# lms-07/LGTEUN

Hardware: AMD Instinct MI355X
Metric: train image-pairs/sec, GF-2 4-band 128x128, K=4, bs=32/GPU (higher is better)
Workload: dtype f32 (GEMMs and the local mixer: split 16-bit MFMA -- f16 pairs in the forward FFN, the W2 products of its backward and P V, bf16 triples elsewhere -- fp32 accumulate; fp32-equivalent); 1 GPU; BASELINE configs[1]: C=4, MS 32x32, PAN 128x128, K=4, 32 pairs/GPU, train step = fwd + L1 + bwd + Adam + StepLR tick; mode=faithful, global_batch=32, parallelism=dp1, dropout=True

## Files before the change

### lgteun_amd/csrc/k_ffn_bwd_x.hip

```cpp
#include "kernels.h"
#include "bwd_kernels.h"
#include "split_bf16.h"
#include "hstore.h"

#ifdef LG_STAMPS
__device__ unsigned long long g_kb_stamps[4 * 16];
#define STAMP(i) do { if (blockIdx.x == 0 && lane == 0 && stamp_on) g_kb_stamps[wave * 16 + (i)] = __builtin_amdgcn_s_memtime(); } while (0)
extern "C" __attribute__((visibility("default"))) int lg_debug_kb_stamps(unsigned long long* host) {
    return (int)hipMemcpyFromSymbol(host, HIP_SYMBOL(g_kb_stamps), sizeof(g_kb_stamps));
}
#else
#define STAMP(i) do { } while (0)
#endif

namespace {

constexpr int NPX = 64;
template <int E>
struct KB {
    static constexpr int N1 = 4 * E, NW = N1 / 16, NT = 64 * NW, LPP = E / 4;
    static constexpr int LDP = N1 + 16;
    static constexpr int D2_PIECE = NPX * LDP;
    static constexpr int XN_PIECE = NPX * E;
    static constexpr int D1T_PIECE = 16 * 16;
    static constexpr size_t OFF_XN = (size_t)3 * D2_PIECE * 2;
    static constexpr size_t OFF_D1T = OFF_XN + (size_t)3 * XN_PIECE * 2;
    static constexpr size_t OFF_RED = OFF_D1T + (size_t)NW * 3 * D1T_PIECE * 2;
    static constexpr size_t LDS_BYTES = OFF_RED + (size_t)NW * NPX * E * 4;
    static constexpr int R_B2 = N1 * N1, R_W1 = R_B2 + N1, R_B1 = R_W1 + N1 * E, R_LG = R_B1 + N1, R_LB = R_LG + E, ROW = R_LB + E;
    static_assert(OFF_XN % 16 == 0 && OFF_D1T % 16 == 0 && OFF_RED % 16 == 0, "16-byte aligned LDS regions");
    static_assert(NT / (N1 / 4) == 16 && NT / LPP == NPX, "loader / LayerNorm thread maps");
};

typedef __attribute__((address_space(3))) s16x4_t lds_s16x4_t;
#ifndef LG_KB_DACHAINS
#define LG_KB_DACHAINS 0
#endif
#ifndef LG_KB_STAGGER
#define LG_KB_STAGGER 0
#endif
#ifndef LG_KB_FENCE
#define LG_KB_FENCE 1
#endif
#define KB_FENCE() do { if (LG_KB_FENCE) __builtin_amdgcn_sched_barrier(0); } while (0)

__device__ __forceinline__ float quad_sum(float v) {
    v += __builtin_bit_cast(float, __builtin_amdgcn_mov_dpp(__builtin_bit_cast(int, v), 0xB1, 0xF, 0xF, true));
    v += __builtin_bit_cast(float, __builtin_amdgcn_mov_dpp(__builtin_bit_cast(int, v), 0x4E, 0xF, 0xF, true));
    return v;
}
__device__ __forceinline__ bf16x8_t lds_x8(const uint16_t* p) { return __builtin_bit_cast(bf16x8_t, *reinterpret_cast<const u32x4_t*>(p)); }
__device__ __forceinline__ s16x4_t lds_x4(const uint16_t* p) { return __builtin_bit_cast(s16x4_t, *reinterpret_cast<const u32x2_t*>(p)); }
__device__ __forceinline__ s16x4_t lds_tr4(const uint16_t* p) {
    return __builtin_amdgcn_ds_read_tr16_b64_v4i16((lds_s16x4_t*)p);
}
__device__ __forceinline__ void mfma6_16(f32x4_t& acc, const s16x4_t (&a)[3], const s16x4_t (&b)[3]) {
    acc = __builtin_amdgcn_mfma_f32_16x16x16bf16_1k(a[0], b[2], acc, 0, 0, 0);
    acc = __builtin_amdgcn_mfma_f32_16x16x16bf16_1k(a[2], b[0], acc, 0, 0, 0);
    acc = __builtin_amdgcn_mfma_f32_16x16x16bf16_1k(a[1], b[1], acc, 0, 0, 0);
    acc = __builtin_amdgcn_mfma_f32_16x16x16bf16_1k(a[0], b[1], acc, 0, 0, 0);
    acc = __builtin_amdgcn_mfma_f32_16x16x16bf16_1k(a[1], b[0], acc, 0, 0, 0);
    acc = __builtin_amdgcn_mfma_f32_16x16x16bf16_1k(a[0], b[0], acc, 0, 0, 0);
}
__device__ __forceinline__ void mfma6_32(f32x4_t& acc, const bf16x8_t (&a)[3], const bf16x8_t (&b)[3]) {
    acc = __builtin_amdgcn_mfma_f32_16x16x32_bf16(a[0], b[2], acc, 0, 0, 0);
    acc = __builtin_amdgcn_mfma_f32_16x16x32_bf16(a[2], b[0], acc, 0, 0, 0);
    acc = __builtin_amdgcn_mfma_f32_16x16x32_bf16(a[1], b[1], acc, 0, 0, 0);
    acc = __builtin_amdgcn_mfma_f32_16x16x32_bf16(a[0], b[1], acc, 0, 0, 0);
    acc = __builtin_amdgcn_mfma_f32_16x16x32_bf16(a[1], b[0], acc, 0, 0, 0);
    acc = __builtin_amdgcn_mfma_f32_16x16x32_bf16(a[0], b[0], acc, 0, 0, 0);
}
__device__ __forceinline__ bf16x8_t cat8(s16x4_t lo, s16x4_t hi) {
    typedef short s16x8_t __attribute__((ext_vector_type(8)));
    return __builtin_bit_cast(bf16x8_t, (s16x8_t)__builtin_shufflevector(lo, hi, 0, 1, 2, 3, 4, 5, 6, 7));
}
#ifndef LG_KB_PAIR
#define LG_KB_PAIR 1
#endif
__device__ __forceinline__ void mfma3_16(f32x4_t& acc, const s16x4_t (&a)[3], const s16x4_t (&b)[3]) {
    const bf16x8_t b31 = cat8(b[2], b[0]), b21 = cat8(b[1], b[0]);
    acc = __builtin_amdgcn_mfma_f32_16x16x32_bf16(cat8(a[0], a[2]), b31, acc, 0, 0, 0);
    acc = __builtin_amdgcn_mfma_f32_16x16x32_bf16(cat8(a[1], a[1]), b21, acc, 0, 0, 0);
    acc = __builtin_amdgcn_mfma_f32_16x16x32_bf16(cat8(a[0], a[0]), b21, acc, 0, 0, 0);
}
template <int NP>
__device__ __forceinline__ void mfmaN_16(f32x4_t& acc, const s16x4_t (&a)[3], const s16x4_t (&b)[3]) {
    if (NP == 3) { if (LG_KB_PAIR) mfma3_16(acc, a, b); else mfma6_16(acc, a, b); }
    else if (NP == 2) {
        const s16x4_t z = {0, 0, 0, 0};
        acc = sb_mfma_h(cat8(a[1], a[0]), cat8(b[0], b[1]), acc);
        acc = sb_mfma_h(cat8(a[0], z), cat8(b[0], z), acc);
    } else acc = __builtin_amdgcn_mfma_f32_16x16x16bf16_1k(a[0], b[0], acc, 0, 0, 0);
}
template <int NP>
__device__ __forceinline__ void mfmaN_32(f32x4_t& acc, const bf16x8_t (&a)[3], const bf16x8_t (&b)[3]) {
    if (NP == 3) mfma6_32(acc, a, b);
    else if (NP == 2) {
        acc = sb_mfma_h(a[1], b[0], acc);
        acc = sb_mfma_h(a[0], b[1], acc);
        acc = sb_mfma_h(a[0], b[0], acc);
    } else acc = __builtin_amdgcn_mfma_f32_16x16x32_bf16(a[0], b[0], acc, 0, 0, 0);
}
template <int NP>
__device__ __forceinline__ void split4(const float (&v)[4], s16x4_t (&p)[3]) {
    u32x2_t q1, q2, q3;
    split_x4<NP>(v, q1, q2, q3);
    p[0] = __builtin_bit_cast(s16x4_t, q1); p[1] = __builtin_bit_cast(s16x4_t, q2); p[2] = __builtin_bit_cast(s16x4_t, q3);
}

template <int NP>
__device__ __forceinline__ void ld3_x4(const uint16_t* p, int piece, s16x4_t (&o)[3]) {
    o[0] = lds_x4(p);
    if (NP == 3) { o[1] = lds_x4(p + piece); o[2] = lds_x4(p + 2 * piece); } else if (NP == 2) { o[1] = lds_x4(p + piece); o[2] = o[0]; } else { o[1] = o[0]; o[2] = o[0]; }
}
template <int NP>
__device__ __forceinline__ void ld3_x8(const uint16_t* p, int piece, bf16x8_t (&o)[3]) {
    o[0] = lds_x8(p);
    if (NP == 3) { o[1] = lds_x8(p + piece); o[2] = lds_x8(p + 2 * piece); } else if (NP == 2) { o[1] = lds_x8(p + piece); o[2] = o[0]; } else { o[1] = o[0]; o[2] = o[0]; }
}
template <int NP>
__device__ __forceinline__ void ld3_tr(const uint16_t* p, int piece, s16x4_t (&o)[3]) {
    o[0] = lds_tr4(p);
    if (NP == 3) { o[1] = lds_tr4(p + piece); o[2] = lds_tr4(p + 2 * piece); } else if (NP == 2) { o[1] = lds_tr4(p + piece); o[2] = o[0]; } else { o[1] = o[0]; o[2] = o[0]; }
}
template <int NP>
__device__ __forceinline__ WFrag32 wfrag32(const float* W, int K, int kb, float ws) { return NP == 3 ? load_wfrag32(W, K, kb) : (NP == 2 ? load_wfrag32_h2(W, K, kb, ws) : load_wfrag32_rne(W, K, kb)); }
template <int NP>
__device__ __forceinline__ WFrag16 wfrag16(const float* W, int K, int k0, float ws) { return NP == 3 ? load_wfrag16(W, K, k0) : (NP == 2 ? load_wfrag16_h2(W, K, k0, ws) : load_wfrag16_rne(W, K, k0)); }
__device__ __forceinline__ float kb_pow2_below(float bound) { return __builtin_amdgcn_ldexpf(1.0f, 15 - __builtin_amdgcn_frexp_expf(bound)); }

template <int E, int NP>
__global__ __launch_bounds__(KB<E>::NT) __attribute__((amdgpu_waves_per_eu(2))) void k_ffn1_bwd_xs(Ffn1BwdXArgs a, long ntiles, int uneven) {
    using C = KB<E>;
    constexpr int N1 = C::N1, NW = C::NW, NT = C::NT, LDP = C::LDP, LPP = C::LPP, D2_PIECE = C::D2_PIECE, XN_PIECE = C::XN_PIECE, D1T_PIECE = C::D1T_PIECE;
    constexpr int KB2 = N1 / 32;
    constexpr int NE = E / 16;
    constexpr bool BF = (NP == 1);
    constexpr int NPE = NP == 2 ? 3 : NP;
    extern __shared__ __attribute__((aligned(16))) unsigned char smem_raw[];
    uint16_t* D2 = reinterpret_cast<uint16_t*>(smem_raw);
    uint16_t* XN = reinterpret_cast<uint16_t*>(smem_raw + C::OFF_XN);
    const int wave = threadIdx.x >> 6, lane = threadIdx.x & 63, r = lane & 15, g = lane >> 4;
    uint16_t* D1T = reinterpret_cast<uint16_t*>(smem_raw + C::OFF_D1T) + wave * 3 * D1T_PIECE;
    float* red = reinterpret_cast<float*>(smem_raw + C::OFF_RED);

    float S_a1 = 1.f, S_w2 = 1.f, S_d2 = 1.f;
    if constexpr (NP == 2) {
        S_a1 = a.scales[1]; S_w2 = a.scales[4];
        S_d2 = kb_pow2_below(fmaxf(a.scales[6], 8.6736174e-19f));
    }
    const float c_d1 = 1.0f / (S_d2 * S_w2);
    WFrag16 w1f16;
    WFrag32 w1f32;
    if constexpr (E == 16) w1f16 = wfrag16<NPE>(a.w1 + (size_t)(wave * 16) * E, E, 0, 1.0f);
    else w1f32 = wfrag32<NPE>(a.w1 + (size_t)(wave * 16) * E, E, 0, 1.0f);
    WFrag32 w2f[KB2];
#pragma unroll
    for (int kb = 0; kb < KB2; ++kb) w2f[kb] = wfrag32<NP>(a.w2t + (size_t)(wave * 16) * N1, N1, kb, S_w2);
    WFrag16 w1tf[NE];
#pragma unroll
    for (int rb = 0; rb < NE; ++rb) w1tf[rb] = wfrag16<NPE>(a.w1t + (size_t)(rb * 16) * N1, N1, wave * 16, 1.0f);
    const float b1s = a.b1[wave * 16 + r];
    const int lpx = threadIdx.x / LPP, lq = threadIdx.x % LPP;
    const float4 lng = *reinterpret_cast<const float4*>(a.ln2g + 4 * lq), lnb = *reinterpret_cast<const float4*>(a.ln2b + 4 * lq);
    const int dq = threadIdx.x % (N1 / 4), dpx = threadIdx.x / (N1 / 4);

    f32x4_t acc2[NW], acc1[NE];
#pragma unroll
    for (int nb = 0; nb < NW; ++nb) acc2[nb] = (f32x4_t){0.f, 0.f, 0.f, 0.f};
#pragma unroll
    for (int cb = 0; cb < NE; ++cb) acc1[cb] = (f32x4_t){0.f, 0.f, 0.f, 0.f};
    float bs1 = 0.f;
    float4 bs2 = make_float4(0.f, 0.f, 0.f, 0.f);
    float4 pg = make_float4(0.f, 0.f, 0.f, 0.f), pb = pg;

    typename HS<BF>::raw4 d2n[4];
    float4 xnx, dyn;
    auto issue = [&](long tile_) {
        const long p0 = tile_ * NPX;
#pragma unroll
        for (int it = 0; it < 4; ++it) d2n[it] = HS<BF>::ldraw(a.dh2, (p0 + dpx + 16 * it) * N1 + 4 * dq);
        xnx = *reinterpret_cast<const float4*>(a.x + (p0 + lpx) * E + 4 * lq);
        dyn = *reinterpret_cast<const float4*>(a.dy + (p0 + lpx) * E + 4 * lq);
    };
    const int half = (int)gridDim.x >> 1, first = (int)blockIdx.x < half ? 1 : 0;
    const long per = uneven ? ntiles / (8 * (long)gridDim.x) : 0;
    const long nmine = uneven ? per * (first ? uneven : 16 - uneven) : (1l << 60);
    const long t0 = uneven ? (first ? (long)blockIdx.x : (long)half * per * uneven + ((long)blockIdx.x - half)) : (long)blockIdx.x;
    const long tstep = uneven ? half : (long)gridDim.x;
    if (t0 < ntiles) issue(t0);

#pragma unroll 1
    for (long tile = t0, kt = 0; tile < ntiles && kt < nmine; tile += tstep, ++kt) {
        const long p0 = tile * NPX;
#ifdef LG_STAMPS
        const bool stamp_on = kt == 2;
#endif
        STAMP(0);
#pragma unroll
        for (int it = 0; it < 4; ++it) {
            const float4 d = HS<BF>::widen(d2n[it]);
            bs2.x += d.x; bs2.y += d.y; bs2.z += d.z; bs2.w += d.w;
            uint16_t* dst = D2 + (dpx + 16 * it) * LDP + 4 * dq;
            if constexpr (BF) {
                *reinterpret_cast<u32x2_t*>(dst) = __builtin_bit_cast(u32x2_t, d2n[it]);
            } else {
                const float v[4] = {d.x * S_d2, d.y * S_d2, d.z * S_d2, d.w * S_d2};
                u32x2_t q1, q2, q3;
                split_x4<NP>(v, q1, q2, q3);
                *reinterpret_cast<u32x2_t*>(dst) = q1;
                *reinterpret_cast<u32x2_t*>(dst + D2_PIECE) = q2;
                if (NP == 3) *reinterpret_cast<u32x2_t*>(dst + 2 * D2_PIECE) = q3;
            }
        }
        const float4 xv = xnx, dyv = dyn;
        const float mu = lane_group_sum<LPP>((xv.x + xv.y) + (xv.z + xv.w)) * (1.0f / E);
        const float c0 = xv.x - mu, c1 = xv.y - mu, c2 = xv.z - mu, c3 = xv.w - mu;
        const float rstd = __builtin_amdgcn_rsqf(lane_group_sum<LPP>((c0 * c0 + c1 * c1) + (c2 * c2 + c3 * c3)) * (1.0f / E) + LG_EPS);
        const float xh[4] = {c0 * rstd, c1 * rstd, c2 * rstd, c3 * rstd};
        {
            const float yv[4] = {xh[0] * lng.x + lnb.x, xh[1] * lng.y + lnb.y, xh[2] * lng.z + lnb.z, xh[3] * lng.w + lnb.w};
            u32x2_t q1, q2, q3;
            split_x4<NPE>(yv, q1, q2, q3);
            uint16_t* dst = XN + lpx * E + 4 * lq;
            *reinterpret_cast<u32x2_t*>(dst) = q1;
            if (NPE == 3) {
                *reinterpret_cast<u32x2_t*>(dst + XN_PIECE) = q2;
                *reinterpret_cast<u32x2_t*>(dst + 2 * XN_PIECE) = q3;
            }
        }
        if (tile + tstep < ntiles && kt + 1 < nmine) issue(tile + tstep);
        STAMP(1);
        __syncthreads();
        STAMP(2);
#if LG_KB_STAGGER
        if (NW == 8 && wave >= 4) __builtin_amdgcn_s_sleep(LG_KB_STAGGER);
#endif

#pragma unroll 1
        for (int pbk = 0; pbk < NPX / 16; ++pbk) {
            f32x4_t h1 = (f32x4_t){b1s, b1s, b1s, b1s};
            if constexpr (E == 16) {
                s16x4_t xa[3];
                ld3_x4<NPE>(XN + (pbk * 16 + r) * E + 4 * g, XN_PIECE, xa);
                KB_FENCE();
                mfmaN_16<NPE>(h1, xa, w1f16.p);
            } else {
                bf16x8_t xa[3];
                ld3_x8<NPE>(XN + (pbk * 16 + r) * E + 8 * g, XN_PIECE, xa);
                KB_FENCE();
                mfmaN_32<NPE>(h1, xa, w1f32.p);
            }
            f32x4_t da = (f32x4_t){0.f, 0.f, 0.f, 0.f};
            {
                const uint16_t* pd = D2 + (pbk * 16 + r) * LDP + 8 * g;
#if LG_KB_DACHAINS
                f32x4_t dak[KB2];
#pragma unroll
                for (int kb = 0; kb < KB2; ++kb) {
                    dak[kb] = (f32x4_t){0.f, 0.f, 0.f, 0.f};
                    bf16x8_t dk[3];
                    ld3_x8<NP>(pd + 32 * kb, D2_PIECE, dk);
                    mfmaN_32<NP>(dak[kb], dk, w2f[kb].p);
                }
#pragma unroll
                for (int kb = 0; kb < KB2; ++kb) da += dak[kb];
#else
#pragma unroll
                for (int kb = 0; kb < KB2; ++kb) {
                    bf16x8_t dk[3];
                    ld3_x8<NP>(pd + 32 * kb, D2_PIECE, dk);
                    mfmaN_32<NP>(da, dk, w2f[kb].p);
                }
#endif
            }
            KB_FENCE();
            lg_v2f a01, a23, g01, g23;
            gelu2_both_t<NP == 1>((lg_v2f){h1[0], h1[1]}, a01, g01);
            gelu2_both_t<NP == 1>((lg_v2f){h1[2], h1[3]}, a23, g23);
            if (NP == 2) { a01 *= S_a1; a23 *= S_a1; g01 *= c_d1; g23 *= c_d1; }
            const float a1v[4] = {a01.x, a01.y, a23.x, a23.y};
            const float d1v[4] = {da[0] * g01.x, da[1] * g01.y, da[2] * g23.x, da[3] * g23.y};
            bs1 += (d1v[0] + d1v[1]) + (d1v[2] + d1v[3]);
            s16x4_t a1p[3], d1p[3];
            split4<NP>(a1v, a1p);
            split4<NPE>(d1v, d1p);
            KB_FENCE();
            {
                const uint16_t* px = XN + (pbk * 16 + 4 * g + (r >> 2)) * E + 4 * (r & 3);
#pragma unroll
                for (int cb = 0; cb < NE; ++cb) {
                    s16x4_t xt[3];
                    ld3_tr<NPE>(px + 16 * cb, XN_PIECE, xt);
                    mfmaN_16<NPE>(acc1[cb], d1p, xt);
                }
                const uint16_t* pt = D2 + (pbk * 16 + 4 * g + (r >> 2)) * LDP + 4 * (r & 3);
#pragma unroll
                for (int nb = 0; nb < NW; ++nb) {
                    s16x4_t dt[3];
                    ld3_tr<NP>(pt + 16 * nb, D2_PIECE, dt);
                    mfmaN_16<NP>(acc2[nb], dt, a1p);
                }
            }
            KB_FENCE();
            {
                uint16_t* dst = D1T + r * 16 + 4 * g;
                *reinterpret_cast<u32x2_t*>(dst) = __builtin_bit_cast(u32x2_t, d1p[0]);
                if (NPE == 3) {
                    *reinterpret_cast<u32x2_t*>(dst + D1T_PIECE) = __builtin_bit_cast(u32x2_t, d1p[1]);
                    *reinterpret_cast<u32x2_t*>(dst + 2 * D1T_PIECE) = __builtin_bit_cast(u32x2_t, d1p[2]);
                }
                __builtin_amdgcn_fence(__ATOMIC_RELEASE, "wavefront");
                __builtin_amdgcn_wave_barrier();
                s16x4_t dtp[3];
                ld3_tr<NPE>(D1T + (4 * g + (r >> 2)) * 16 + 4 * (r & 3), D1T_PIECE, dtp);
#pragma unroll
                for (int rb = 0; rb < NE; ++rb) {
                    f32x4_t o = (f32x4_t){0.f, 0.f, 0.f, 0.f};
                    mfmaN_16<NPE>(o, w1tf[rb].p, dtp);
                    *reinterpret_cast<float4*>(red + ((size_t)wave * NPX + pbk * 16 + r) * E + 16 * rb + 4 * g) = make_float4(o[0], o[1], o[2], o[3]);
                }
                __builtin_amdgcn_wave_barrier();
            }
        }
        STAMP(3);
        __syncthreads();
        STAMP(4);

        {
            const float* rp = red + (size_t)lpx * E + 4 * lq;
            float dl[4] = {0.f, 0.f, 0.f, 0.f};
#pragma unroll
            for (int w2 = 0; w2 < NW; w2 += 2) {
                const float4 s0 = *reinterpret_cast<const float4*>(rp + (size_t)w2 * NPX * E), s1 = *reinterpret_cast<const float4*>(rp + (size_t)(w2 + 1) * NPX * E);
                dl[0] += s0.x + s1.x; dl[1] += s0.y + s1.y; dl[2] += s0.z + s1.z; dl[3] += s0.w + s1.w;
            }
            pg.x += dl[0] * xh[0]; pg.y += dl[1] * xh[1]; pg.z += dl[2] * xh[2]; pg.w += dl[3] * xh[3];
            pb.x += dl[0]; pb.y += dl[1]; pb.z += dl[2]; pb.w += dl[3];
            const float dxh[4] = {dl[0] * lng.x, dl[1] * lng.y, dl[2] * lng.z, dl[3] * lng.w};
            const float m1 = lane_group_sum<LPP>((dxh[0] + dxh[1]) + (dxh[2] + dxh[3])) * (1.0f / E);
            const float m2 = lane_group_sum<LPP>((dxh[0] * xh[0] + dxh[1] * xh[1]) + (dxh[2] * xh[2] + dxh[3] * xh[3])) * (1.0f / E);
            *reinterpret_cast<float4*>(a.dx + (p0 + lpx) * E + 4 * lq) =
                make_float4(dyv.x + rstd * (dxh[0] - m1 - xh[0] * m2), dyv.y + rstd * (dxh[1] - m1 - xh[1] * m2),
                            dyv.z + rstd * (dxh[2] - m1 - xh[2] * m2), dyv.w + rstd * (dxh[3] - m1 - xh[3] * m2));
        }
        STAMP(5);
    }

    float* row = a.slab + (size_t)blockIdx.x * C::ROW;
    const float inv_w2 = 1.0f / (S_d2 * S_a1);
#pragma unroll
    for (int nb = 0; nb < NW; ++nb)
#pragma unroll
        for (int v = 0; v < 4; ++v) row[(16 * nb + 4 * g + v) * N1 + 16 * wave + r] = acc2[nb][v] * inv_w2;
#pragma unroll
    for (int cb = 0; cb < NE; ++cb)
#pragma unroll
        for (int v = 0; v < 4; ++v) row[C::R_W1 + (16 * wave + 4 * g + v) * E + 16 * cb + r] = acc1[cb][v];
    {
        float s = bs1;
        s += __shfl_xor(s, 16);
        s += __shfl_xor(s, 32);
        if (g == 0) row[C::R_B1 + 16 * wave + r] = s;
    }
    __syncthreads();
    float* sc = reinterpret_cast<float*>(smem_raw);
    *reinterpret_cast<float4*>(sc + dpx * N1 + 4 * dq) = bs2;
    *reinterpret_cast<float4*>(sc + 16 * N1 + lpx * E + 4 * lq) = pg;
    *reinterpret_cast<float4*>(sc + 16 * N1 + NPX * E + lpx * E + 4 * lq) = pb;
    __syncthreads();
    if (threadIdx.x < N1) {
        float s = 0.f;
#pragma unroll
        for (int k = 0; k < 16; ++k) s += sc[k * N1 + threadIdx.x];
        row[C::R_B2 + threadIdx.x] = s;
    } else if (threadIdx.x < N1 + 2 * E) {
        const int i = threadIdx.x - N1, which = i / E, c = i % E;
        const float* src = sc + 16 * N1 + which * NPX * E + c;
        float s = 0.f;
        for (int k = 0; k < NPX; ++k) s += src[k * E];
        row[(which ? C::R_LB : C::R_LG) + c] = s;
    }
}

template <int E>
int launch_t(const Ffn1BwdXArgs& a, hipStream_t s) {
    using C = KB<E>;
    static DeviceOnce attr_once;
    if (attr_once.need()) {
        hipError_t e = hipFuncSetAttribute((const void*)k_ffn1_bwd_xs<E, 3>, hipFuncAttributeMaxDynamicSharedMemorySize, (int)C::LDS_BYTES);
        if (e == hipSuccess) e = hipFuncSetAttribute((const void*)k_ffn1_bwd_xs<E, 1>, hipFuncAttributeMaxDynamicSharedMemorySize, (int)C::LDS_BYTES);
        if (e == hipSuccess) e = hipFuncSetAttribute((const void*)k_ffn1_bwd_xs<E, 2>, hipFuncAttributeMaxDynamicSharedMemorySize, (int)C::LDS_BYTES);
        if (e != hipSuccess) { lg_set_error("ffn1_bwd_xs: hipFuncSetAttribute: %s", hipGetErrorString(e)); return (int)e; }
        attr_once.done();
    }
    const long ntiles = a.P / NPX;
    const int cap = ffn1_bwd_x_wgs(E);
    const int grid = (int)(ntiles < cap ? ntiles : cap);
#ifndef LG_FFN1B_UNEVEN
#define LG_FFN1B_UNEVEN 9
#endif
    const int uneven = (E == 16 && grid == 512 && ntiles % (8 * (long)grid) == 0 && LG_FFN1B_UNEVEN != 8) ? LG_FFN1B_UNEVEN : 0;
    if (a.hbf) k_ffn1_bwd_xs<E, 1><<<grid, C::NT, C::LDS_BYTES, s>>>(a, ntiles, uneven);
    else if (a.scales) k_ffn1_bwd_xs<E, 2><<<grid, C::NT, C::LDS_BYTES, s>>>(a, ntiles, uneven);
    else k_ffn1_bwd_xs<E, 3><<<grid, C::NT, C::LDS_BYTES, s>>>(a, ntiles, uneven);
    LG_CHECK_LAUNCH();
    ReduceJob j;
    j.dst2 = nullptr; j.nslices = grid; j.slice_stride = C::ROW;
    auto job = [&](int off, float* dst, int rows, int cols) {
        j.slab = a.slab + off; j.dst = dst; j.rows = rows; j.cols = cols; j.row_stride = cols; j.ld = cols; j.rows_valid = rows; j.cols_valid = cols;
        return launch_reduce_job(j, s);
    };
    int rc = job(0, a.d_w2, C::N1, C::N1);
    if (!rc) rc = job(C::R_B2, a.d_b2, 1, C::N1);
    if (!rc) rc = job(C::R_W1, a.d_w1, C::N1, E);
    if (!rc) rc = job(C::R_B1, a.d_b1, 1, C::N1);
    if (!rc) rc = job(C::R_LG, a.d_ln2g, 1, E);
    if (!rc) rc = job(C::R_LB, a.d_ln2b, 1, E);
    return rc;
}

}

size_t ffn1_bwd_x_slab_floats(int e) { return (size_t)ffn1_bwd_x_wgs(e) * (e == 16 ? KB<16>::ROW : KB<32>::ROW); }

int launch_ffn1_bwd_xs(int e, const Ffn1BwdXArgs& a, hipStream_t s) {
    ProfScope prof__(LG_K_FFN1_BWD, s);
    if (e != 16 && e != 32) { lg_set_error("ffn1_bwd_xs: e=%d unsupported", e); return -1; }
    if (a.P <= 0 || a.P % NPX) { lg_set_error("ffn1_bwd_xs: pixel count %ld is not a multiple of %d", a.P, NPX); return -2; }
    if (!a.dh2 || !a.x || !a.dy || !a.dx || !a.slab || !a.w1 || !a.w1t || !a.w2t || !a.b1 || !a.ln2g || !a.ln2b) { lg_set_error("ffn1_bwd_xs: null argument"); return -2; }
    if (e == 32) return launch_t<32>(a, s);
    return launch_t<16>(a, s);
}
```

### lgteun_amd/csrc/k_ffn_dwbwd_x.hip

```cpp
#include "kernels.h"
#include "bwd_kernels.h"
#include "split_bf16.h"
#include "hstore.h"

#ifdef LG_STAMPS
__device__ unsigned long long g_ka_stamps[8 * 16];
#define STAMP(i) do { if (blockIdx.x == 0 && lane == 0 && stamp_on) g_ka_stamps[wave * 16 + (i)] = __builtin_amdgcn_s_memtime(); } while (0)
extern "C" __attribute__((visibility("default"))) int lg_debug_ka_stamps(unsigned long long* host) {
    return (int)hipMemcpyFromSymbol(host, HIP_SYMBOL(g_ka_stamps), sizeof(g_ka_stamps));
}
#else
#define STAMP(i) do { } while (0)
#endif

namespace {

constexpr int TX = 16, HX = 18, TY = 8, RING = 10, CH = 48;
constexpr int NH = 64, NW = 4, NT = 256, LDR = NH + 4, CQ = NH / 4;
constexpr int A3_PIECE = 16 * 16;
template <int E_>
struct KA {
    static constexpr int E = E_, N1 = 4 * E, NHALF = N1 / NH, LQ = E / 4, NV = (CH * LQ + NT - 1) / NT;
    static constexpr int DY_PIECE = CH * E;
    static constexpr int DY_SLOT = 3 * DY_PIECE;
    static constexpr size_t OFF_DY = (size_t)RING * HX * LDR * 4;
    static constexpr size_t OFF_A3 = OFF_DY + (size_t)2 * DY_SLOT * 2;
    static constexpr size_t OFF_TAPS = OFF_A3 + (size_t)NW * 3 * A3_PIECE * 2;
    static constexpr size_t LDS_BYTES = OFF_TAPS + (size_t)NH * 9 * 4;
    static constexpr int R_DB = NH * 9, R_W3 = NH * 10, R_B3 = R_W3 + E * NH, ROW = R_B3 + E;
    static_assert(OFF_DY % 16 == 0 && OFF_A3 % 16 == 0 && OFF_TAPS % 16 == 0, "16-byte aligned LDS regions");
    static_assert((size_t)(NW * CQ * 40 + NW * E) * 4 <= OFF_DY, "the end-of-kernel reduction rows alias the ring");
    static_assert(LDS_BYTES <= 80 * 1024, "two workgroups per CU");
};
static_assert(KA<16>::R_DB == FFN_DW_BWD_X_DB && KA<16>::R_W3 == FFN_DW_BWD_X_W3 && KA<16>::R_B3 == FFN_DW_BWD_X_B3 && KA<16>::ROW == FFN_DW_BWD_X_ROW, "slab row (bwd_kernels.h)");
static_assert(KA<32>::ROW == FFN_DW_BWD_X32_ROW, "slab row (bwd_kernels.h)");

typedef __attribute__((address_space(3))) s16x4_t lds_s16x4_t;
__device__ __forceinline__ s16x4_t lds_x4(const uint16_t* p) { return __builtin_bit_cast(s16x4_t, *reinterpret_cast<const u32x2_t*>(p)); }
__device__ __forceinline__ s16x4_t lds_tr4(const uint16_t* p) { return __builtin_amdgcn_ds_read_tr16_b64_v4i16((lds_s16x4_t*)p); }
__device__ __forceinline__ void mfma6_16(f32x4_t& acc, const s16x4_t (&a)[3], const s16x4_t (&b)[3]) {
    acc = __builtin_amdgcn_mfma_f32_16x16x16bf16_1k(a[0], b[2], acc, 0, 0, 0);
    acc = __builtin_amdgcn_mfma_f32_16x16x16bf16_1k(a[2], b[0], acc, 0, 0, 0);
    acc = __builtin_amdgcn_mfma_f32_16x16x16bf16_1k(a[1], b[1], acc, 0, 0, 0);
    acc = __builtin_amdgcn_mfma_f32_16x16x16bf16_1k(a[0], b[1], acc, 0, 0, 0);
    acc = __builtin_amdgcn_mfma_f32_16x16x16bf16_1k(a[1], b[0], acc, 0, 0, 0);
    acc = __builtin_amdgcn_mfma_f32_16x16x16bf16_1k(a[0], b[0], acc, 0, 0, 0);
}

__device__ __forceinline__ bf16x8_t cat8(s16x4_t lo, s16x4_t hi) {
    typedef short s16x8_t __attribute__((ext_vector_type(8)));
    return __builtin_bit_cast(bf16x8_t, (s16x8_t)__builtin_shufflevector(lo, hi, 0, 1, 2, 3, 4, 5, 6, 7));
}
#ifndef LG_KA_ITEMFENCE
#define LG_KA_ITEMFENCE 1
#endif
#ifndef LG_KA_PAIR
#define LG_KA_PAIR 0
#endif
__device__ __forceinline__ void mfma3_16(f32x4_t& acc, const s16x4_t (&a)[3], const s16x4_t (&b)[3]) {
    const bf16x8_t b31 = cat8(b[2], b[0]), b21 = cat8(b[1], b[0]);
    acc = __builtin_amdgcn_mfma_f32_16x16x32_bf16(cat8(a[0], a[2]), b31, acc, 0, 0, 0);
    acc = __builtin_amdgcn_mfma_f32_16x16x32_bf16(cat8(a[1], a[1]), b21, acc, 0, 0, 0);
    acc = __builtin_amdgcn_mfma_f32_16x16x32_bf16(cat8(a[0], a[0]), b21, acc, 0, 0, 0);
}
template <int NP>
__device__ __forceinline__ void mfmaN_16(f32x4_t& acc, const s16x4_t (&a)[3], const s16x4_t (&b)[3]) {
    if (NP == 3) { if (LG_KA_PAIR) mfma3_16(acc, a, b); else mfma6_16(acc, a, b); }
    else acc = __builtin_amdgcn_mfma_f32_16x16x16bf16_1k(a[0], b[0], acc, 0, 0, 0);
}

__device__ __forceinline__ bf16x8_t lds_x8(const uint16_t* p) { return __builtin_bit_cast(bf16x8_t, *reinterpret_cast<const u32x4_t*>(p)); }

template <int E, int NP>
__global__ __launch_bounds__(NT) __attribute__((amdgpu_waves_per_eu(2))) void k_ffn_dw_bwd_xs(FfnDwBwdXArgs a, int tiles_x, int strips_y, int nstrips, int SH, int dS) {
    using C = KA<E>;
    constexpr int N1 = C::N1, LQ = C::LQ, NV = C::NV, DY_PIECE = C::DY_PIECE, DY_SLOT = C::DY_SLOT;
    constexpr int PPL = 4, RPW = 2, NM = E / 16;
    constexpr bool BF = (NP == 1);
    const int hoff = blockIdx.y * NH;
    extern __shared__ __attribute__((aligned(16))) unsigned char smem_raw[];
    float* ring = reinterpret_cast<float*>(smem_raw);
    uint16_t* DY = reinterpret_cast<uint16_t*>(smem_raw + C::OFF_DY);
    const int wave = threadIdx.x >> 6, lane = threadIdx.x & 63, r = lane & 15, g = lane >> 4;
    uint16_t* A3 = reinterpret_cast<uint16_t*>(smem_raw + C::OFF_A3) + wave * 3 * A3_PIECE;
    const int h = a.h, w = a.w;
    const int c0 = wave * 16 + 4 * g;
    WFrag16 w3f16;
    WFrag32 w3f32;
    if constexpr (E == 16) w3f16 = NP == 3 ? load_wfrag16(a.w3t + (size_t)(hoff + wave * 16) * E, E, 0) : load_wfrag16_rne(a.w3t + (size_t)(hoff + wave * 16) * E, E, 0);
    else w3f32 = NP == 3 ? load_wfrag32(a.w3t + (size_t)(hoff + wave * 16) * E, E, 0) : load_wfrag32_rne(a.w3t + (size_t)(hoff + wave * 16) * E, E, 0);
    const int q = lane % CQ, lgrp = lane / CQ;
    const int lq = threadIdx.x % LQ;
    auto dy_px = [&](int v) { return (threadIdx.x + NT * v) / LQ; };
    auto dy_has = [&](int v) { return threadIdx.x + NT * v < LQ * CH; };

    float* sTaps = reinterpret_cast<float*>(smem_raw + C::OFF_TAPS);
    for (int i = threadIdx.x; i < NH * 9; i += NT) sTaps[i] = a.dww[hoff * 9 + i];
    lg_v2f pw01[10], pw23[10];
#pragma unroll
    for (int k = 0; k < 10; ++k) { pw01[k] = (lg_v2f){0.f, 0.f}; pw23[k] = (lg_v2f){0.f, 0.f}; }
    f32x4_t acc3[NM];
#pragma unroll
    for (int mt = 0; mt < NM; ++mt) acc3[mt] = (f32x4_t){0.f, 0.f, 0.f, 0.f};
    float4 sb3 = make_float4(0.f, 0.f, 0.f, 0.f);

    float dmx = 0.f;
#pragma unroll 1
    for (int strip = blockIdx.x; strip < nstrips; strip += gridDim.x) {
    int tx_i, Y0, Yend;
    long b;
    if (dS) {
        const int half = nstrips >> 1, shortone = strip >= half ? 1 : 0;
        int p_ = strip - (shortone ? half : 0);
        tx_i = p_ % tiles_x;
        p_ /= tiles_x;
        const int hy2 = strips_y >> 1, ky = p_ % hy2;
        b = p_ / hy2;
        Y0 = ky * 2 * SH + (shortone ? SH + dS : 0);
        Yend = min(Y0 + (shortone ? SH - dS : SH + dS), h);
    } else {
        int t = strip;
        tx_i = t % tiles_x;
        t /= tiles_x;
        const int sy = t % strips_y;
        b = t / strips_y;
        Y0 = sy * SH;
        Yend = min(Y0 + SH, h);
    }
    const int x0 = tx_i * TX;
#ifdef LG_STAMPS
    bool stamp_on = false;
#endif

    struct DyVec { float4 dv[NV]; bool in[NV], own[NV]; };
    auto dy_fetch = [&](int ya, int npx, int c, DyVec& d) {
#pragma unroll
        for (int v = 0; v < NV; ++v) {
            const int m = c * CH + dy_px(v);
            const int hy = m / HX, hx = m - hy * HX;
            const int y = ya + hy, x = x0 + hx - 1;
            d.in[v] = dy_has(v) && (m < npx) && y >= 0 && y < h && x >= 0 && x < w;
            d.own[v] = d.in[v] && hx >= 1 && hx <= TX && y >= Y0 && y < Yend;
            d.dv[v] = *reinterpret_cast<const float4*>(a.dy + ((b * h + clampi(y, 0, h - 1)) * (long)w + clampi(x, 0, w - 1)) * E + 4 * lq);
        }
    };
    auto dy_store = [&](int slot, const DyVec& d) {
#pragma unroll
        for (int v = 0; v < NV; ++v) {
            const float4 dvr = d.dv[v];
            const bool in = d.in[v];
            const float4 dv = make_float4(in ? dvr.x : 0.f, in ? dvr.y : 0.f, in ? dvr.z : 0.f, in ? dvr.w : 0.f);
            if (d.own[v]) { sb3.x += dv.x; sb3.y += dv.y; sb3.z += dv.z; sb3.w += dv.w; }
            if (!dy_has(v)) continue;
            const float vv[4] = {dv.x, dv.y, dv.z, dv.w};
            u32x2_t q1, q2, q3;
            split_x4<NP>(vv, q1, q2, q3);
            uint16_t* dst = DY + slot * DY_SLOT + dy_px(v) * E + 4 * lq;
            *reinterpret_cast<u32x2_t*>(dst) = q1;
            if (NP == 3) {
                *reinterpret_cast<u32x2_t*>(dst + DY_PIECE) = q2;
                *reinterpret_cast<u32x2_t*>(dst + 2 * DY_PIECE) = q3;
            }
        }
    };
    auto h3_fetch = [&](int ya, int c, typename HS<BF>::raw4 (&hv)[3]) {
#pragma unroll
        for (int pb = 0; pb < 3; ++pb) {
            const int m = c * CH + pb * 16 + r;
            const int hy = m / HX, hx = m - hy * HX;
            const int y = clampi(ya + hy, 0, h - 1), x = clampi(x0 + hx - 1, 0, w - 1);
            hv[pb] = HS<BF>::ldraw(a.h3, ((b * h + y) * (long)w + x) * N1 + hoff + c0);
        }
    };

    auto compute_rows = [&](int ya, int nr, const DyVec& pre, typename HS<BF>::raw4 (&h3c)[3], auto&& in_last) {
        const int npx = nr * HX, nchunks = (npx + CH - 1) / CH;
        typename HS<BF>::raw4 h3n[3];
        dy_store(0, pre);
        STAMP(1);
        __syncthreads();
        STAMP(2);
        const int ring0 = ((ya - Y0 + 1) % RING) * HX;
        for (int c = 0; c < nchunks; ++c) {
            const int slot = c & 1;
            const bool more = c + 1 < nchunks;
            DyVec nd;
            if (more) { dy_fetch(ya, npx, c + 1, nd); h3_fetch(ya, c + 1, h3n); }
            else in_last();
            const uint16_t* dyb = DY + slot * DY_SLOT;
#pragma unroll
            for (int pb = 0; pb < 3; ++pb) {
                const int m = c * CH + pb * 16 + r;
                const int hy = m / HX, hx = m - hy * HX;
                const int y = ya + hy, x = x0 + hx - 1;
                const bool own = m < npx && hx >= 1 && hx <= TX && x < w && y >= Y0 && y < Yend;
                f32x4_t acc = (f32x4_t){0.f, 0.f, 0.f, 0.f};
                if constexpr (E == 16) {
                    const uint16_t* p = dyb + (pb * 16 + r) * E + 4 * g;
                    s16x4_t xb[3];
                    xb[0] = lds_x4(p);
                    if (NP == 3) { xb[1] = lds_x4(p + DY_PIECE); xb[2] = lds_x4(p + 2 * DY_PIECE); } else { xb[1] = xb[0]; xb[2] = xb[0]; }
                    mfmaN_16<NP>(acc, w3f16.p, xb);
                } else {
                    const uint16_t* p = dyb + (pb * 16 + r) * E + 8 * g;
                    const bf16x8_t x1 = lds_x8(p);
                    bf16x8_t x2 = x1, x3 = x1;
                    if (NP == 3) { x2 = lds_x8(p + DY_PIECE); x3 = lds_x8(p + 2 * DY_PIECE); }
                    mfma_np32<NP>(acc, w3f32, x1, x2, x3);
                }
                lg_v2f a01, a23, g01, g23;
                const float4 h3v = HS<BF>::widen(h3c[pb]);
                gelu2_both_t<NP == 1>((lg_v2f){h3v.x, h3v.y}, a01, g01);
                gelu2_both_t<NP == 1>((lg_v2f){h3v.z, h3v.w}, a23, g23);
                int rp = ring0 + m;
                rp = rp >= RING * HX ? rp - RING * HX : rp;
                if (m < npx) *reinterpret_cast<float4*>(ring + rp * LDR + c0) = make_float4(acc[0] * g01.x, acc[1] * g01.y, acc[2] * g23.x, acc[3] * g23.y);
                const float mk = own ? 1.0f : 0.0f;
                const float av[4] = {a01.x * mk, a01.y * mk, a23.x * mk, a23.y * mk};
                u32x2_t q1, q2, q3;
                split_x4<NP>(av, q1, q2, q3);
                uint16_t* dst = A3 + r * 16 + 4 * g;
                *reinterpret_cast<u32x2_t*>(dst) = q1;
                if (NP == 3) {
                    *reinterpret_cast<u32x2_t*>(dst + A3_PIECE) = q2;
                    *reinterpret_cast<u32x2_t*>(dst + 2 * A3_PIECE) = q3;
                }
                __builtin_amdgcn_fence(__ATOMIC_RELEASE, "wavefront");
                __builtin_amdgcn_wave_barrier();
                {
                    const uint16_t* pbp = A3 + (4 * g + (r >> 2)) * 16 + 4 * (r & 3);
                    s16x4_t at[3];
                    at[0] = lds_tr4(pbp);
                    if (NP == 3) { at[1] = lds_tr4(pbp + A3_PIECE); at[2] = lds_tr4(pbp + 2 * A3_PIECE); } else { at[1] = at[0]; at[2] = at[0]; }
#pragma unroll
                    for (int mt = 0; mt < NM; ++mt) {
                        const uint16_t* pa = dyb + (pb * 16 + 4 * g + (r >> 2)) * E + 16 * mt + 4 * (r & 3);
                        s16x4_t dt[3];
                        dt[0] = lds_tr4(pa);
                        if (NP == 3) { dt[1] = lds_tr4(pa + DY_PIECE); dt[2] = lds_tr4(pa + 2 * DY_PIECE); } else { dt[1] = dt[0]; dt[2] = dt[0]; }
                        mfmaN_16<NP>(acc3[mt], dt, at);
                    }
                }
                __builtin_amdgcn_wave_barrier();
            }
            if (more) {
                dy_store(slot ^ 1, nd);
#pragma unroll
                for (int pb = 0; pb < 3; ++pb) h3c[pb] = h3n[pb];
            }
            STAMP(3 + 2 * c);
            __syncthreads();
            STAMP(4 + 2 * c);
        }
    };

    DyVec pre;
    typename HS<BF>::raw4 h3p[3];
    dy_fetch(Y0 - 1, 2 * HX, 0, pre);
    h3_fetch(Y0 - 1, 0, h3p);
    DyVec npre;
    typename HS<BF>::raw4 nh3[3];
    compute_rows(Y0 - 1, 2, pre, h3p, [&] { dy_fetch(Y0 + 1, TY * HX, 0, npre); h3_fetch(Y0 + 1, 0, nh3); });
#pragma unroll 1
    for (int y0 = Y0; y0 < Yend; y0 += TY) {
#ifdef LG_STAMPS
        stamp_on = (y0 == Y0 + 2 * TY) && strip == 0;
#endif
        STAMP(0);
        const int yrow0 = y0 + RPW * wave, xl0 = x0 + PPL * lgrp;
        auto h2_at = [&](int y, int x) { return HS<BF>::ldraw(a.h2, ((b * h + y) * (long)w + x) * N1 + hoff + 4 * q); };
        typename HS<BF>::raw4 h2a, h2b, h2c, h2d;
        pre = npre;
#pragma unroll
        for (int pb = 0; pb < 3; ++pb) h3p[pb] = nh3[pb];
        compute_rows(y0 + 1, TY, pre, h3p, [&] { h2a = h2_at(yrow0, xl0); h2b = h2_at(yrow0, xl0 + 1); h2c = h2_at(yrow0, xl0 + 2); h2d = h2_at(yrow0, xl0 + 3); });
        lg_v2f wq01[9], wq23[9];
        {
            const float* tp = sTaps + 36 * q;
            float t36[36];
#pragma unroll
            for (int k4 = 0; k4 < 9; ++k4) {
                const float4 v = *reinterpret_cast<const float4*>(tp + 4 * k4);
                t36[4 * k4] = v.x; t36[4 * k4 + 1] = v.y; t36[4 * k4 + 2] = v.z; t36[4 * k4 + 3] = v.w;
            }
#pragma unroll
            for (int k = 0; k < 9; ++k) { wq01[k] = (lg_v2f){t36[k], t36[9 + k]}; wq23[k] = (lg_v2f){t36[18 + k], t36[27 + k]}; }
        }
        __builtin_amdgcn_sched_barrier(0);
        dy_fetch(y0 + TY + 1, TY * HX, 0, npre);
        h3_fetch(y0 + TY + 1, 0, nh3);
        STAMP(9);
        const int sbase = (y0 - Y0) % RING;
        auto rowN = [&](int ch) {
            const int ty = RPW * wave + ch, y = y0 + ty, txb = PPL * lgrp;
            const float* rrow[3];
#pragma unroll
            for (int rr = 0; rr < 3; ++rr) {
                int sl = sbase + ty + rr;
                sl = sl >= RING ? sl - RING : sl;
                rrow[rr] = ring + (sl * HX + txb) * LDR + 4 * q;
            }
            float4 col[4][3];
            auto ldcol = [&](int c) {
#pragma unroll
                for (int rr = 0; rr < 3; ++rr) col[c & 3][rr] = *reinterpret_cast<const float4*>(rrow[rr] + c * LDR);
            };
            ldcol(0); ldcol(1); ldcol(2);
            auto item = [&](int it, typename HS<BF>::raw4& hreg) {
                if (it + 1 < PPL) ldcol(it + 3);
                const int x = x0 + txb + it;
                const float4 hc = HS<BF>::widen(hreg);
                {
                    const int nit = it + 4, ny = nit < PPL ? y : (ch + 1 < RPW ? y + 1 : y), nx = x0 + txb + (nit < PPL ? nit : nit - PPL);
                    hreg = h2_at(ny, nx);
                }
                const lg_v2f h01 = (lg_v2f){hc.x, hc.y}, h23 = (lg_v2f){hc.z, hc.w};
                lg_v2f acc01 = (lg_v2f){0.f, 0.f}, acc23 = (lg_v2f){0.f, 0.f};
#pragma unroll
                for (int rr = 0; rr < 3; ++rr)
#pragma unroll
                    for (int cc = 0; cc < 3; ++cc) {
                        const int k = (2 - rr) * 3 + (2 - cc);
                        const float4 gv = col[(it + cc) & 3][rr];
                        const lg_v2f g01 = (lg_v2f){gv.x, gv.y}, g23 = (lg_v2f){gv.z, gv.w};
                        acc01 = wq01[k] * g01 + acc01;
                        acc23 = wq23[k] * g23 + acc23;
                        pw01[k] = h01 * g01 + pw01[k];
                        pw23[k] = h23 * g23 + pw23[k];
                        if (k == 4) { pw01[9] += g01; pw23[9] += g23; }
                    }
                HS<BF>::st4(a.dh2, ((b * h + y) * (long)w + x) * N1 + hoff + 4 * q, make_float4(acc01.x, acc01.y, acc23.x, acc23.y));
                if (NP != 1) dmx = fmaxf(fmaxf(dmx, fmaxf(fabsf(acc01.x), fabsf(acc01.y))), fmaxf(fabsf(acc23.x), fabsf(acc23.y)));
                if (LG_KA_ITEMFENCE && ((it + 1) % LG_KA_ITEMFENCE) == 0) __builtin_amdgcn_sched_barrier(0);
            };
            item(0, h2a); item(1, h2b); item(2, h2c); item(3, h2d);
        };
#pragma unroll 1
        for (int ch = 0; ch < RPW; ++ch) rowN(ch);
        STAMP(10);
    }
    __syncthreads();
    }

    if (NP != 1 && a.dh2_max) {
#pragma unroll
        for (int off = 32; off > 0; off >>= 1) dmx = fmaxf(dmx, __shfl_xor(dmx, off));
        if (lane == 0) atomicMax(reinterpret_cast<unsigned int*>(a.dh2_max), __float_as_uint(dmx));
    }
    float* row = a.slab + ((size_t)blockIdx.y * gridDim.x + blockIdx.x) * C::ROW;
#pragma unroll
    for (int mt = 0; mt < NM; ++mt)
#pragma unroll
        for (int v = 0; v < 4; ++v) row[C::R_W3 + (16 * mt + 4 * g + v) * NH + 16 * wave + r] = acc3[mt][v];
    float* red = ring;
#pragma unroll
    for (int u = 0; u < 4; ++u)
#pragma unroll
        for (int k = 0; k < 10; ++k) {
            float v = u == 0 ? pw01[k].x : (u == 1 ? pw01[k].y : (u == 2 ? pw23[k].x : pw23[k].y));
#pragma unroll
            for (int off = CQ; off < 64; off <<= 1) v += __shfl_xor(v, off);
            if (lane < CQ) red[(wave * CQ + q) * 40 + u * 10 + k] = v;
        }
    {
        float4 s4 = sb3;
#pragma unroll
        for (int off = LQ; off < 64; off <<= 1) {
            s4.x += __shfl_xor(s4.x, off); s4.y += __shfl_xor(s4.y, off); s4.z += __shfl_xor(s4.z, off); s4.w += __shfl_xor(s4.w, off);
        }
        if (lane < LQ) *reinterpret_cast<float4*>(red + NW * CQ * 40 + wave * E + 4 * lane) = s4;
    }
    __syncthreads();
    for (int i = threadIdx.x; i < CQ * 40; i += NT) {
        float v = 0.f;
#pragma unroll
        for (int w8 = 0; w8 < NW; ++w8) v += red[w8 * CQ * 40 + i];
        const int qq = i / 40, rem = i - qq * 40, u = rem / 10, k = rem - u * 10;
        const int c = 4 * qq + u;
        if (k < 9) row[c * 9 + k] = v;
        else row[C::R_DB + c] = v;
    }
    if (threadIdx.x < E) {
        const float* sp = red + NW * CQ * 40 + threadIdx.x;
        float v = 0.f;
#pragma unroll
        for (int w8 = 0; w8 < NW; ++w8) v += sp[w8 * E];
        row[C::R_B3 + threadIdx.x] = v;
    }
}

template <int E>
static int launch_dw_t(const FfnDwBwdXArgs& a, hipStream_t s) {
    using C = KA<E>;
    static DeviceOnce attr_once;
    if (attr_once.need()) {
        hipError_t e = hipFuncSetAttribute((const void*)k_ffn_dw_bwd_xs<E, 3>, hipFuncAttributeMaxDynamicSharedMemorySize, (int)C::LDS_BYTES);
        if (e == hipSuccess) e = hipFuncSetAttribute((const void*)k_ffn_dw_bwd_xs<E, 1>, hipFuncAttributeMaxDynamicSharedMemorySize, (int)C::LDS_BYTES);
        if (e != hipSuccess) { lg_set_error("ffn_dw_bwd_xs: hipFuncSetAttribute: %s", hipGetErrorString(e)); return (int)e; }
        attr_once.done();
    }
    const int tiles_x = (a.w + 15) / 16;
    const int wgs = FFN_DW_BWD_X_WGS / C::NHALF;
    int SH = (a.h + 7) / 8 * 8;
    while (SH > 16 && (long)a.B * tiles_x * ((a.h + SH - 1) / SH) < wgs) SH = (SH / 2 + 7) / 8 * 8;
    const int strips_y = (a.h + SH - 1) / SH;
    const int nstrips = a.B * tiles_x * strips_y;
    const int gx = nstrips < wgs ? nstrips : wgs;
    const dim3 grid(gx, C::NHALF);
#ifndef LG_DWB_UNEVEN
#define LG_DWB_UNEVEN 0
#endif
    int dS = 0;
    if (LG_DWB_UNEVEN && E == 16 && nstrips == wgs && wgs == 512 && (strips_y & 1) == 0 && SH >= 32 && a.h % (2 * SH) == 0) dS = (SH * LG_DWB_UNEVEN / 64 + 7) / 8 * 8;
    if (a.hbf) k_ffn_dw_bwd_xs<E, 1><<<grid, NT, C::LDS_BYTES, s>>>(a, tiles_x, strips_y, nstrips, SH, dS);
    else k_ffn_dw_bwd_xs<E, 3><<<grid, NT, C::LDS_BYTES, s>>>(a, tiles_x, strips_y, nstrips, SH, dS);
    LG_CHECK_LAUNCH();
    ReduceJob j;
    j.dst2 = nullptr; j.nslices = gx; j.slice_stride = C::ROW;
    int rc = 0;
    for (int half = 0; half < C::NHALF && !rc; ++half) {
        const float* base = a.slab + (size_t)half * gx * C::ROW;
        auto job = [&](int off, float* dst, int rows, int cols, int ld) {
            j.slab = base + off; j.dst = dst; j.rows = rows; j.cols = cols; j.row_stride = cols; j.ld = ld; j.rows_valid = rows; j.cols_valid = cols;
            return launch_reduce_job(j, s);
        };
        rc = job(0, a.d_dww + (size_t)half * NH * 9, NH, 9, 9);
        if (!rc) rc = job(C::R_DB, a.d_dwb + half * NH, 1, NH, NH);
        if (!rc) rc = job(C::R_W3, a.d_w3 + half * NH, E, NH, C::N1);
        if (!rc && half == 0) rc = job(C::R_B3, a.d_b3, 1, E, E);
    }
    return rc;
}

}

int launch_ffn_dw_bwd_xs(int e, const FfnDwBwdXArgs& a, hipStream_t s) {
    ProfScope prof__(LG_K_FFN2_BWD, s);
    if (e != 16 && e != 32) { lg_set_error("ffn_dw_bwd_xs: e=%d unsupported", e); return -1; }
    if (!a.dy || !a.h3 || !a.h2 || !a.dh2 || !a.w3t || !a.dww || !a.slab) { lg_set_error("ffn_dw_bwd_xs: null argument"); return -2; }
    if ((a.h & 7) || (a.w & 15)) { lg_set_error("ffn_dw_bwd_xs: h must be a multiple of 8 and w of 16 (got %d x %d)", a.h, a.w); return -2; }
    return e == 16 ? launch_dw_t<16>(a, s) : launch_dw_t<32>(a, s);
}
```

Measured before the change: 6257 image-pairs/sec.

## XOR-swizzle LDS layouts in FFN backward kernels to avoid bank conflicts

Adds XOR swizzle helpers for the staged activation, gradient, transpose-scratch and reduction buffers in the two FFN backward kernels. Every store and load site, including transposed reads, is rewritten to use the permuted offsets, with the offsets precomputed per lane. The goal is to remove LDS bank conflicts on the strided row and column accesses. It also remaps the lane-to-channel assignment in the dw reduction so it needs fewer shuffles. The risk is that any mismatch between the store and load permutations silently corrupts gradients.

```diff
diff --git a/lgteun_amd/csrc/k_ffn_bwd_x.hip b/lgteun_amd/csrc/k_ffn_bwd_x.hip
--- a/lgteun_amd/csrc/k_ffn_bwd_x.hip
+++ b/lgteun_amd/csrc/k_ffn_bwd_x.hip
@@ -2,6 +2,7 @@
 #include "bwd_kernels.h"
 #include "split_bf16.h"
 #include "hstore.h"
+#include "lds_swizzle.h"
 
 #ifdef LG_STAMPS
 __device__ unsigned long long g_kb_stamps[4 * 16];
@@ -143,6 +144,7 @@
     const int wave = threadIdx.x >> 6, lane = threadIdx.x & 63, r = lane & 15, g = lane >> 4;
     uint16_t* D1T = reinterpret_cast<uint16_t*>(smem_raw + C::OFF_D1T) + wave * 3 * D1T_PIECE;
     float* red = reinterpret_cast<float*>(smem_raw + C::OFF_RED);
+    const int xnr_off = lds_rowcol<E>(r, (E / 16) * g), xnt_off = lds_rowcol<E>(4 * g + (r >> 2), r & 3), red_off = lds_red<E>(r, g);
 
     float S_a1 = 1.f, S_w2 = 1.f, S_d2 = 1.f;
     if constexpr (NP == 2) {
@@ -222,7 +224,7 @@
             const float yv[4] = {xh[0] * lng.x + lnb.x, xh[1] * lng.y + lnb.y, xh[2] * lng.z + lnb.z, xh[3] * lng.w + lnb.w};
             u32x2_t q1, q2, q3;
             split_x4<NPE>(yv, q1, q2, q3);
-            uint16_t* dst = XN + lpx * E + 4 * lq;
+            uint16_t* dst = XN + lds_rowcol<E>(lpx, lq);
             *reinterpret_cast<u32x2_t*>(dst) = q1;
             if (NPE == 3) {
                 *reinterpret_cast<u32x2_t*>(dst + XN_PIECE) = q2;
@@ -242,12 +244,12 @@
             f32x4_t h1 = (f32x4_t){b1s, b1s, b1s, b1s};
             if constexpr (E == 16) {
                 s16x4_t xa[3];
-                ld3_x4<NPE>(XN + (pbk * 16 + r) * E + 4 * g, XN_PIECE, xa);
+                ld3_x4<NPE>(XN + pbk * 16 * E + xnr_off, XN_PIECE, xa);
                 KB_FENCE();
                 mfmaN_16<NPE>(h1, xa, w1f16.p);
             } else {
                 bf16x8_t xa[3];
-                ld3_x8<NPE>(XN + (pbk * 16 + r) * E + 8 * g, XN_PIECE, xa);
+                ld3_x8<NPE>(XN + pbk * 16 * E + xnr_off, XN_PIECE, xa);
                 KB_FENCE();
                 mfmaN_32<NPE>(h1, xa, w1f32.p);
             }
@@ -287,11 +289,11 @@
             split4<NPE>(d1v, d1p);
             KB_FENCE();
             {
-                const uint16_t* px = XN + (pbk * 16 + 4 * g + (r >> 2)) * E + 4 * (r & 3);
+                const uint16_t* px = XN + pbk * 16 * E;
 #pragma unroll
                 for (int cb = 0; cb < NE; ++cb) {
                     s16x4_t xt[3];
-                    ld3_tr<NPE>(px + 16 * cb, XN_PIECE, xt);
+                    ld3_tr<NPE>(px + (xnt_off ^ (16 * cb)), XN_PIECE, xt);
                     mfmaN_16<NPE>(acc1[cb], d1p, xt);
                 }
                 const uint16_t* pt = D2 + (pbk * 16 + 4 * g + (r >> 2)) * LDP + 4 * (r & 3);
@@ -304,7 +306,7 @@
             }
             KB_FENCE();
             {
-                uint16_t* dst = D1T + r * 16 + 4 * g;
+                uint16_t* dst = D1T + lds_img16(r, g);
                 *reinterpret_cast<u32x2_t*>(dst) = __builtin_bit_cast(u32x2_t, d1p[0]);
                 if (NPE == 3) {
                     *reinterpret_cast<u32x2_t*>(dst + D1T_PIECE) = __builtin_bit_cast(u32x2_t, d1p[1]);
@@ -313,12 +315,12 @@
                 __builtin_amdgcn_fence(__ATOMIC_RELEASE, "wavefront");
                 __builtin_amdgcn_wave_barrier();
                 s16x4_t dtp[3];
-                ld3_tr<NPE>(D1T + (4 * g + (r >> 2)) * 16 + 4 * (r & 3), D1T_PIECE, dtp);
+                ld3_tr<NPE>(D1T + lds_img16(4 * g + (r >> 2), r & 3), D1T_PIECE, dtp);
 #pragma unroll
                 for (int rb = 0; rb < NE; ++rb) {
                     f32x4_t o = (f32x4_t){0.f, 0.f, 0.f, 0.f};
                     mfmaN_16<NPE>(o, w1tf[rb].p, dtp);
-                    *reinterpret_cast<float4*>(red + ((size_t)wave * NPX + pbk * 16 + r) * E + 16 * rb + 4 * g) = make_float4(o[0], o[1], o[2], o[3]);
+                    *reinterpret_cast<float4*>(red + (wave * NPX + pbk * 16) * E + (red_off ^ (16 * rb))) = make_float4(o[0], o[1], o[2], o[3]);
                 }
                 __builtin_amdgcn_wave_barrier();
             }
@@ -328,7 +330,7 @@
         STAMP(4);
 
         {
-            const float* rp = red + (size_t)lpx * E + 4 * lq;
+            const float* rp = red + lds_red<E>(lpx, lq);
             float dl[4] = {0.f, 0.f, 0.f, 0.f};
 #pragma unroll
             for (int w2 = 0; w2 < NW; w2 += 2) {
diff --git a/lgteun_amd/csrc/k_ffn_dwbwd_x.hip b/lgteun_amd/csrc/k_ffn_dwbwd_x.hip
--- a/lgteun_amd/csrc/k_ffn_dwbwd_x.hip
+++ b/lgteun_amd/csrc/k_ffn_dwbwd_x.hip
@@ -2,6 +2,7 @@
 #include "bwd_kernels.h"
 #include "split_bf16.h"
 #include "hstore.h"
+#include "lds_swizzle.h"
 
 #ifdef LG_STAMPS
 __device__ unsigned long long g_ka_stamps[8 * 16];
@@ -89,10 +90,11 @@
     WFrag32 w3f32;
     if constexpr (E == 16) w3f16 = NP == 3 ? load_wfrag16(a.w3t + (size_t)(hoff + wave * 16) * E, E, 0) : load_wfrag16_rne(a.w3t + (size_t)(hoff + wave * 16) * E, E, 0);
     else w3f32 = NP == 3 ? load_wfrag32(a.w3t + (size_t)(hoff + wave * 16) * E, E, 0) : load_wfrag32_rne(a.w3t + (size_t)(hoff + wave * 16) * E, E, 0);
-    const int q = lane % CQ, lgrp = lane / CQ;
+    const int q = (lane & 3) | ((lane >> 1) & 12), lgrp = ((lane >> 5) << 1) | (((lane >> 2) ^ (lane >> 3) ^ (lane >> 4)) & 1);
     const int lq = threadIdx.x % LQ;
     auto dy_px = [&](int v) { return (threadIdx.x + NT * v) / LQ; };
     auto dy_has = [&](int v) { return threadIdx.x + NT * v < LQ * CH; };
+    const int dys_off = lds_rowcol<E>(dy_px(0), lq), dyr_off = lds_rowcol<E>(r, (E / 16) * g), dyt_off = lds_rowcol<E>(4 * g + (r >> 2), r & 3);
 
     float* sTaps = reinterpret_cast<float*>(smem_raw + C::OFF_TAPS);
     for (int i = threadIdx.x; i < NH * 9; i += NT) sTaps[i] = a.dww[hoff * 9 + i];
@@ -155,7 +157,7 @@
             const float vv[4] = {dv.x, dv.y, dv.z, dv.w};
             u32x2_t q1, q2, q3;
             split_x4<NP>(vv, q1, q2, q3);
-            uint16_t* dst = DY + slot * DY_SLOT + dy_px(v) * E + 4 * lq;
+            uint16_t* dst = DY + slot * DY_SLOT + dys_off + v * (NT / LQ) * E;
             *reinterpret_cast<u32x2_t*>(dst) = q1;
             if (NP == 3) {
                 *reinterpret_cast<u32x2_t*>(dst + DY_PIECE) = q2;
@@ -196,13 +198,13 @@
                 const bool own = m < npx && hx >= 1 && hx <= TX && x < w && y >= Y0 && y < Yend;
                 f32x4_t acc = (f32x4_t){0.f, 0.f, 0.f, 0.f};
                 if constexpr (E == 16) {
-                    const uint16_t* p = dyb + (pb * 16 + r) * E + 4 * g;
+                    const uint16_t* p = dyb + pb * 16 * E + dyr_off;
                     s16x4_t xb[3];
                     xb[0] = lds_x4(p);
                     if (NP == 3) { xb[1] = lds_x4(p + DY_PIECE); xb[2] = lds_x4(p + 2 * DY_PIECE); } else { xb[1] = xb[0]; xb[2] = xb[0]; }
                     mfmaN_16<NP>(acc, w3f16.p, xb);
                 } else {
-                    const uint16_t* p = dyb + (pb * 16 + r) * E + 8 * g;
+                    const uint16_t* p = dyb + pb * 16 * E + dyr_off;
                     const bf16x8_t x1 = lds_x8(p);
                     bf16x8_t x2 = x1, x3 = x1;
                     if (NP == 3) { x2 = lds_x8(p + DY_PIECE); x3 = lds_x8(p + 2 * DY_PIECE); }
@@ -219,7 +221,7 @@
                 const float av[4] = {a01.x * mk, a01.y * mk, a23.x * mk, a23.y * mk};
                 u32x2_t q1, q2, q3;
                 split_x4<NP>(av, q1, q2, q3);
-                uint16_t* dst = A3 + r * 16 + 4 * g;
+                uint16_t* dst = A3 + lds_img16(r, g);
                 *reinterpret_cast<u32x2_t*>(dst) = q1;
                 if (NP == 3) {
                     *reinterpret_cast<u32x2_t*>(dst + A3_PIECE) = q2;
@@ -228,13 +230,13 @@
                 __builtin_amdgcn_fence(__ATOMIC_RELEASE, "wavefront");
                 __builtin_amdgcn_wave_barrier();
                 {
-                    const uint16_t* pbp = A3 + (4 * g + (r >> 2)) * 16 + 4 * (r & 3);
+                    const uint16_t* pbp = A3 + lds_img16(4 * g + (r >> 2), r & 3);
                     s16x4_t at[3];
                     at[0] = lds_tr4(pbp);
                     if (NP == 3) { at[1] = lds_tr4(pbp + A3_PIECE); at[2] = lds_tr4(pbp + 2 * A3_PIECE); } else { at[1] = at[0]; at[2] = at[0]; }
 #pragma unroll
                     for (int mt = 0; mt < NM; ++mt) {
-                        const uint16_t* pa = dyb + (pb * 16 + 4 * g + (r >> 2)) * E + 16 * mt + 4 * (r & 3);
+                        const uint16_t* pa = dyb + pb * 16 * E + (dyt_off ^ (16 * mt));
                         s16x4_t dt[3];
                         dt[0] = lds_tr4(pa);
                         if (NP == 3) { dt[1] = lds_tr4(pa + DY_PIECE); dt[2] = lds_tr4(pa + 2 * DY_PIECE); } else { dt[1] = dt[0]; dt[2] = dt[0]; }
@@ -358,9 +360,9 @@
 #pragma unroll
         for (int k = 0; k < 10; ++k) {
             float v = u == 0 ? pw01[k].x : (u == 1 ? pw01[k].y : (u == 2 ? pw23[k].x : pw23[k].y));
-#pragma unroll
-            for (int off = CQ; off < 64; off <<= 1) v += __shfl_xor(v, off);
-            if (lane < CQ) red[(wave * CQ + q) * 40 + u * 10 + k] = v;
+            v += __shfl_xor(v, 4);
+            v += __shfl_xor(v, 32);
+            if (lgrp == 0) red[(wave * CQ + q) * 40 + u * 10 + k] = v;
         }
     {
         float4 s4 = sb3;
diff --git a/lgteun_amd/csrc/lds_swizzle.h b/lgteun_amd/csrc/lds_swizzle.h
--- /dev/null
+++ b/lgteun_amd/csrc/lds_swizzle.h
@@ -0,0 +1,15 @@
+#pragma once
+
+__device__ __forceinline__ int lds_img16(int r, int c) { return r * 16 + 4 * (c ^ ((r >> 2) & 3)); }
+
+template <int E>
+__device__ __forceinline__ int lds_rowcol(int px, int j) {
+    if (E == 16) return px * 16 + 4 * (j ^ (((px >> 3) & 1) << 1));
+    return px * 32 + 4 * (j ^ (((0x78 >> (2 * ((px >> 2) & 3))) & 3) << 1));
+}
+
+template <int E>
+__device__ __forceinline__ int lds_red(int px, int c) {
+    if (E == 16) return px * 16 + 4 * (c ^ ((px >> 1) & 3));
+    return px * 32 + 4 * (c ^ (px & 7));
+}
```

Result: no change. 6292 image-pairs/sec (median of 6 runs) (+0.6%).
